# psy-ex/svt-av1-psy

Measured on AMD Instinct MI355X. Metric: Mblocks/s per kernel (SAD, FwdTxfm2d, CDEF) + encoder fps @1080p preset 8, higher is better.
Workload: dtype u8

## Files before the change

### svt-av1-psy_amd/csrc/sad.hip

```cpp
#include "svt_hip_common.h"
#include "../../include/svtav1_hip.h"
#include "hme_geom.h"
#include <vector>

namespace {

struct __attribute__((packed, aligned(4))) U64A4 { unsigned long long v; };
struct __attribute__((aligned(4))) u32x4_a4 { uint32_t x, y, z, w; };
struct __attribute__((aligned(16))) u32x4_a16 { uint32_t x, y, z, w; };

constexpr uint32_t MAX_SAD_VALUE = 128 * 128 * 255;
constexpr int      ME_TW         = 64;
constexpr int      ME_TH         = 32;
constexpr int      KEY_POS_BITS  = 11;
constexpr uint32_t ME_WAVE_MAX_W = 24, ME_WAVE_MAX_H = 16;

__device__ __forceinline__ void stage_rows_u8(uint32_t* lds, int pitch_dw, const uint8_t* g, uint32_t gstride, int width,
                                              int rows, int tid, int nthreads) {
    const int total = rows * pitch_dw;
    for (int i = tid; i < total; i += nthreads) {
        const int r   = i / pitch_dw;
        const int k   = i - r * pitch_dw;
        const int col = k * 4;
        uint32_t  v   = 0;
        if (col < width) {
            const uint8_t*  p    = g + (size_t)r * gstride + col;
            const uint32_t  sh   = (uint32_t)((uintptr_t)p & 3);
            const uint32_t* ap   = (const uint32_t*)(p - sh);
            const int       need = (width - col) < 4 ? (width - col) : 4;
            const uint32_t  lo   = ap[0];
            uint32_t        hi   = 0;
            if ((int)sh + need > 4) hi = ap[1];
            v = __builtin_amdgcn_alignbyte(hi, lo, sh);
            if (need < 4) v &= (1u << (8 * need)) - 1u;
        }
        lds[i] = v;
    }
}

struct __attribute__((packed, aligned(1))) u32x4_a1 { uint32_t x, y, z, w; };
struct __attribute__((packed, aligned(1))) u32_a1 { uint32_t x; };
struct __attribute__((aligned(8))) u32x2_a8 { uint32_t x, y; };

template <int NIT, int CL2>
__device__ __forceinline__ void stage_rows_load(uint32_t (&v)[NIT][4], const uint8_t* g, uint32_t gstride, int width, int rows, int tid) {
#pragma unroll
    for (int k = 0; k < NIT; ++k) {
        const int  idx = tid + 256 * k, r = idx >> CL2, col = (idx & ((1 << CL2) - 1)) * 16;
        const bool live = r < rows && col < width;
        const int  left = width - col;
        const int  back = (live && left < 16) ? 16 - left : 0;
        const uint8_t* p = g + (live ? (size_t)r * gstride + (size_t)(col - back) : (size_t)0);
        const u32x4_a1 t = *(const u32x4_a1*)p;
        v[k][0] = t.x; v[k][1] = t.y; v[k][2] = t.z; v[k][3] = t.w;
    }
#pragma unroll
    for (int k = 0; k < NIT; ++k) {
        const int  idx = tid + 256 * k, r = idx >> CL2, col = (idx & ((1 << CL2) - 1)) * 16;
        const bool live = r < rows && col < width;
        const int  left = width - col;
        uint32_t   x0 = live ? v[k][0] : 0u, x1 = live ? v[k][1] : 0u, x2 = live ? v[k][2] : 0u, x3 = live ? v[k][3] : 0u;
        if (live && left < 16) {
            const int back = 16 - left;
            if (back & 4) { x0 = x1; x1 = x2; x2 = x3; x3 = 0; }
            if (back & 8) { x0 = x2; x1 = x3; x2 = 0; x3 = 0; }
            const uint32_t bs = (uint32_t)back & 3u;
            x0 = __builtin_amdgcn_alignbyte(x1, x0, bs);
            x1 = __builtin_amdgcn_alignbyte(x2, x1, bs);
            x2 = __builtin_amdgcn_alignbyte(x3, x2, bs);
            x3 = __builtin_amdgcn_alignbyte(0u, x3, bs);
        }
        v[k][0] = x0; v[k][1] = x1; v[k][2] = x2; v[k][3] = x3;
    }
}
template <int NIT, int CL2>
__device__ __forceinline__ void stage_rows_store(const uint32_t (&v)[NIT][4], uint32_t* lds, int pitch_dw, int rows, int tid) {
#pragma unroll
    for (int k = 0; k < NIT; ++k) {
        const int idx = tid + 256 * k, r = idx >> CL2, c4 = (idx & ((1 << CL2) - 1)) * 4;
        if (r < rows) {
            uint32_t* o = lds + r * pitch_dw + c4;
            if (c4 + 0 < pitch_dw) *(u32x2_a8*)(o + 0) = u32x2_a8{v[k][0], v[k][1]};
            if (c4 + 2 < pitch_dw) *(u32x2_a8*)(o + 2) = u32x2_a8{v[k][2], v[k][3]};
        }
    }
}

template <int NT, int U>
__device__ __forceinline__ void stage_rows_wide_step(uint32_t* lds, const int pitch_dw, const uint8_t* g, const uint32_t gstride, const int width, const int total,
                                                     const int cpr, const int dr, const int dc, const int base, const int tid, int& r, int& c) {
    uint32_t v[U][4];
    int      rk[U], ck[U];
#pragma unroll
    for (int k = 0; k < U; ++k) {
        const int  idx = base + tid + NT * k, col = c * 16;
        rk[k] = r; ck[k] = c;
        const bool live = idx < total && col < width;
        const int  left = width - col;
        const int  back = (live && left < 16) ? 16 - left : 0;
        const uint8_t* p = g + (live ? (uint32_t)r * gstride + (uint32_t)(col - back) : 0u);
        const u32x4_a1 t = *(const u32x4_a1*)p;
        uint32_t x0 = live ? t.x : 0u, x1 = live ? t.y : 0u, x2 = live ? t.z : 0u, x3 = live ? t.w : 0u;
        if (back) {
            if (back & 4) { x0 = x1; x1 = x2; x2 = x3; x3 = 0; }
            if (back & 8) { x0 = x2; x1 = x3; x2 = 0; x3 = 0; }
            const uint32_t bs = (uint32_t)back & 3u;
            x0 = __builtin_amdgcn_alignbyte(x1, x0, bs);
            x1 = __builtin_amdgcn_alignbyte(x2, x1, bs);
            x2 = __builtin_amdgcn_alignbyte(x3, x2, bs);
            x3 = __builtin_amdgcn_alignbyte(0u, x3, bs);
        }
        v[k][0] = x0; v[k][1] = x1; v[k][2] = x2; v[k][3] = x3;
        r += dr; c += dc;
        if (c >= cpr) { c -= cpr; r++; }
    }
#pragma unroll
    for (int k = 0; k < U; ++k) {
        const int idx = base + tid + NT * k, c4 = ck[k] * 4;
        if (idx < total) {
            uint32_t* o = lds + rk[k] * pitch_dw + c4;
            if (c4 + 0 < pitch_dw) *(u32x2_a8*)(o + 0) = u32x2_a8{v[k][0], v[k][1]};
            if (c4 + 2 < pitch_dw) *(u32x2_a8*)(o + 2) = u32x2_a8{v[k][2], v[k][3]};
        }
    }
}
template <int NT = 256>
__device__ __forceinline__ void stage_rows_wide_any(uint32_t* lds, int pitch_dw, const uint8_t* g, uint32_t gstride, int width, int rows, int tid) {
    const int cpr = (pitch_dw + 3) >> 2, total = rows * cpr;
    const int dr = NT / cpr, dc = NT - dr * cpr;
    int       r = tid / cpr, c = tid - r * cpr;
    int base = 0;
    for (; total - base > 2 * NT; base += 4 * NT) stage_rows_wide_step<NT, 4>(lds, pitch_dw, g, gstride, width, total, cpr, dr, dc, base, tid, r, c);
    if (total - base > NT) stage_rows_wide_step<NT, 2>(lds, pitch_dw, g, gstride, width, total, cpr, dr, dc, base, tid, r, c);
    else if (total - base > 0) stage_rows_wide_step<NT, 1>(lds, pitch_dw, g, gstride, width, total, cpr, dr, dc, base, tid, r, c);
}

template <int NT>
__device__ __forceinline__ void stage_rows_wide_cpr(uint32_t* lds, int pitch_dw, const uint8_t* g, uint32_t gstride, int width, int rows, int cpr, int tid) {
    const int total = rows * cpr, dr = NT / cpr, dc = NT - dr * cpr;
    int       r = tid / cpr, c = tid - r * cpr, base = 0;
    for (; total - base > 2 * NT; base += 4 * NT) stage_rows_wide_step<NT, 4>(lds, pitch_dw, g, gstride, width, total, cpr, dr, dc, base, tid, r, c);
    if (total - base > NT) stage_rows_wide_step<NT, 2>(lds, pitch_dw, g, gstride, width, total, cpr, dr, dc, base, tid, r, c);
    else if (total - base > 0) stage_rows_wide_step<NT, 1>(lds, pitch_dw, g, gstride, width, total, cpr, dr, dc, base, tid, r, c);
}

__device__ __forceinline__ uint32_t dpp_add_quad_xor1(uint32_t v) {
    return v + (uint32_t)__builtin_amdgcn_update_dpp(0, (int)v, 0xB1, 0xf, 0xf, false);
}
__device__ __forceinline__ uint32_t dpp_add_quad_xor2(uint32_t v) {
    return v + (uint32_t)__builtin_amdgcn_update_dpp(0, (int)v, 0x4E, 0xf, 0xf, false);
}
__device__ __forceinline__ uint32_t dpp_add_row_ror4(uint32_t v) {
    return v + (uint32_t)__builtin_amdgcn_update_dpp(0, (int)v, 0x124, 0xf, 0xf, false);
}
__device__ __forceinline__ uint32_t dpp_add_row_ror8(uint32_t v) {
    return v + (uint32_t)__builtin_amdgcn_update_dpp(0, (int)v, 0x128, 0xf, 0xf, false);
}
__device__ __forceinline__ uint32_t umin32(uint32_t a, uint32_t b) { return a < b ? a : b; }


constexpr int ME_PITCH = 34;

template <bool SUB, bool FULL, int PITCH = ME_PITCH>
__device__ __forceinline__ void me_search_strips(const uint32_t* __restrict__ win, const uint32_t (&s)[8][2], int Wt, int Ht, int g0, int gstep, int l,
                                                 uint32_t& best8, uint32_t& best16, uint32_t& best32, uint32_t& best64) {
    const int bx = (l & 1) | ((l >> 1) & 2) | ((l >> 2) & 4);
    const int by = ((l >> 1) & 1) | ((l >> 2) & 2) | ((l >> 3) & 4);
    const int q  = l & 3;
    const int      G    = (Wt + 3) >> 2;
    const uint32_t qsel = 0x0c0c0100u + 0x0202u * (uint32_t)q;
    for (int g = g0; g < G; g += gstep) {
        const uint32_t* colp   = win + (by * 8) * PITCH + bx * 2 + g;
        const int       nvalid = (Wt - 4 * g) < 4 ? (Wt - 4 * g) : 4;
        const uint32_t inv1 = nvalid > 1 ? 0u : 0xffffffffu, inv2 = nvalid > 2 ? 0u : 0xffffffffu, inv3 = nvalid > 3 ? 0u : 0xffffffffu;
        const uint32_t invq = q < nvalid ? 0u : 0xffffffffu;
        U64A4 ra[8], rb[8];
#pragma unroll
        for (int r = 0; r < 7; r++) {
            ra[r] = *(const U64A4*)(colp + r * PITCH);
            rb[r] = *(const U64A4*)(colp + r * PITCH + 1);
        }
        uint32_t pos = (uint32_t)(4 * g), posq = (uint32_t)(4 * g + q);
        for (int yb = 0; yb < Ht; yb += 8) {
            const uint32_t* rowp = colp + (yb + 7) * PITCH;
#pragma unroll
            for (int i = 0; i < 8; i++) {
                if (yb + i < Ht) {
                    ra[(i + 7) & 7] = *(const U64A4*)(rowp + i * PITCH);
                    rb[(i + 7) & 7] = *(const U64A4*)(rowp + i * PITCH + 1);
                    unsigned long long acc = 0;
#pragma unroll
                    for (int r = 0; r < 8; r += (SUB ? 2 : 1)) {
                        acc = __builtin_amdgcn_qsad_pk_u16_u8(ra[(i + r) & 7].v, s[r][0], acc);
                        acc = __builtin_amdgcn_qsad_pk_u16_u8(rb[(i + r) & 7].v, s[r][1], acc);
                    }
                    if (SUB) acc <<= 1;
                    const uint32_t lo = (uint32_t)acc, hi = (uint32_t)(acc >> 32);
                    uint32_t k0 = (lo << 16) | pos, k1 = (lo & 0xffff0000u) | (pos + 1), k2 = (hi << 16) | (pos + 2),
                             k3 = (hi & 0xffff0000u) | (pos + 3);
                    if (!FULL) { k1 |= inv1; k2 |= inv2; k3 |= inv3; }
                    best8 = umin32(umin32(best8, k0), k1);
                    best8 = umin32(umin32(best8, k2), k3);
                    const uint32_t tlo = dpp_add_quad_xor2(dpp_add_quad_xor1(lo));
                    const uint32_t thi = dpp_add_quad_xor2(dpp_add_quad_xor1(hi));
                    const uint32_t sad16 = __builtin_amdgcn_perm(thi, tlo, qsel);
                    const uint32_t pq    = FULL ? posq : (posq | invq);
                    best16 = umin32(best16, (sad16 << KEY_POS_BITS) | pq);
                    const uint32_t sad32 = dpp_add_row_ror8(dpp_add_row_ror4(sad16));
                    best32 = umin32(best32, (sad32 << KEY_POS_BITS) | pq);
                    const auto     x16   = __builtin_amdgcn_permlane16_swap(sad32, sad32, false, false);
                    const uint32_t pair  = x16[0] + x16[1];
                    const auto     x32   = __builtin_amdgcn_permlane32_swap(pair, pair, false, false);
                    const uint32_t sad64 = x32[0] + x32[1];
                    best64 = umin32(best64, (sad64 << KEY_POS_BITS) | pq);
                    pos += ME_TW;
                    posq += ME_TW;
                }
            }
        }
    }
}

template <bool SUB>
__global__ __launch_bounds__(256, 4) void me_fullpel_kernel(const uint8_t* __restrict__ src_base, const uint8_t* __restrict__ ref_base,
                                                         const SvtHipMeSearchDesc* __restrict__ descs, uint32_t n,
                                                         uint32_t tiles_x,
                                                         uint32_t* __restrict__ best_sad, uint32_t* __restrict__ best_mv,
                                                         unsigned long long* __restrict__ keys) {
    HIP_DYNAMIC_SHARED(uint32_t, smem)
    uint32_t* src_lds  = smem;
    uint32_t* best_lds = smem + 64 * 16;
    uint32_t* win      = smem + 64 * 16 + 88;

    const int      tid  = threadIdx.x;
    const uint32_t item = xcd_remap(blockIdx.x, n);
    const uint32_t tile = blockIdx.y;
    const SvtHipMeSearchDesc d = descs[item];
    const int W   = d.search_area_width, H = d.search_area_height;
    const int tx0 = (int)(tile % tiles_x) * ME_TW;
    const int ty0 = (int)(tile / tiles_x) * ME_TH;
    if (tx0 >= W || ty0 >= H) {
        if (tile == 0 && keys == nullptr && tid < SVT_HIP_ME_NUM_BLOCKS) {
            best_sad[(size_t)item * SVT_HIP_ME_NUM_BLOCKS + tid] = MAX_SAD_VALUE;
            best_mv[(size_t)item * SVT_HIP_ME_NUM_BLOCKS + tid]  = 0;
        }
        return;
    }
    const int Wt = (W - tx0) < ME_TW ? (W - tx0) : ME_TW;
    const int Ht = (H - ty0) < ME_TH ? (H - ty0) : ME_TH;

    {
        uint32_t vs[1][4], vw[3][4];
        stage_rows_load<1, 2>(vs, src_base + d.src_off, d.src_stride, 64, 64, tid);
        stage_rows_load<3, 3>(vw, ref_base + d.ref_off + (size_t)ty0 * d.ref_stride + tx0, d.ref_stride, 64 + Wt - 1, 64 + Ht - 1, tid);
        stage_rows_store<1, 2>(vs, src_lds, 16, 64, tid);
        stage_rows_store<3, 3>(vw, win, ME_PITCH, 64 + Ht - 1, tid);
    }
    if (tid < 88) best_lds[tid] = 0xffffffffu;
    __syncthreads();

    const int l  = tid & 63;
    const int wv = tid >> 6;
    uint32_t s[8][2];
    {
        const int bx = (l & 1) | ((l >> 1) & 2) | ((l >> 2) & 4);
        const int by = ((l >> 1) & 1) | ((l >> 2) & 2) | ((l >> 3) & 4);
#pragma unroll
        for (int r = 0; r < 8; r++) {
            s[r][0] = src_lds[(by * 8 + r) * 16 + bx * 2 + 0];
            s[r][1] = src_lds[(by * 8 + r) * 16 + bx * 2 + 1];
        }
    }
    uint32_t best8 = 0xffffffffu, best16 = 0xffffffffu, best32 = 0xffffffffu, best64 = 0xffffffffu;
    if ((Wt & 3) == 0) me_search_strips<SUB, true>(win, s, Wt, Ht, wv, 4, l, best8, best16, best32, best64);
    else me_search_strips<SUB, false>(win, s, Wt, Ht, wv, 4, l, best8, best16, best32, best64);

    atomicMin(&best_lds[21 + l], best8);
    atomicMin(&best_lds[5 + (l >> 2)], best16);
    atomicMin(&best_lds[1 + (l >> 4)], best32);
    atomicMin(&best_lds[0], best64);
    __syncthreads();
    if (tid < SVT_HIP_ME_NUM_BLOCKS) {
        const uint32_t key = best_lds[tid];
        const uint32_t sad = tid >= 21 ? (key >> 16) : (key >> KEY_POS_BITS);
        const int      X   = tx0 + (int)(key & 63u);
        const int      Y   = ty0 + (int)((key >> 6) & 31u);
        const size_t   o   = (size_t)item * SVT_HIP_ME_NUM_BLOCKS + tid;
        if (keys == nullptr) {
            best_sad[o] = sad;
            best_mv[o]  = ((uint32_t)(uint16_t)(Y + d.y_search_area_origin) << 16) | (uint16_t)(X + d.x_search_area_origin);
        } else {
            atomicMin(&keys[o], ((unsigned long long)sad << 32) | (unsigned long long)(uint32_t)(Y * W + X));
        }
    }
}

struct __attribute__((packed, aligned(1))) u32x2_a1 { uint32_t x, y; };
__device__ __forceinline__ uint32_t dpp_min_quad_xor1(uint32_t v) { return umin32(v, (uint32_t)__builtin_amdgcn_update_dpp(-1, (int)v, 0xB1, 0xf, 0xf, false)); }
__device__ __forceinline__ uint32_t dpp_min_quad_xor2(uint32_t v) { return umin32(v, (uint32_t)__builtin_amdgcn_update_dpp(-1, (int)v, 0x4E, 0xf, 0xf, false)); }
__device__ __forceinline__ uint32_t dpp_min_row_ror4(uint32_t v) { return umin32(v, (uint32_t)__builtin_amdgcn_update_dpp(-1, (int)v, 0x124, 0xf, 0xf, false)); }
__device__ __forceinline__ uint32_t dpp_min_row_ror8(uint32_t v) { return umin32(v, (uint32_t)__builtin_amdgcn_update_dpp(-1, (int)v, 0x128, 0xf, 0xf, false)); }

template <bool SUB, int PITCH>
__global__ __launch_bounds__(256) void me_fullpel_wave_kernel(const uint8_t* __restrict__ src_base, const uint8_t* __restrict__ ref_base,
                                                              const SvtHipMeSearchDesc* __restrict__ descs, const uint32_t n, const int win_dw,
                                                              uint32_t* __restrict__ best_sad, uint32_t* __restrict__ best_mv) {
    HIP_DYNAMIC_SHARED(uint32_t, smem)
    const int      l    = threadIdx.x & 63, wv = __builtin_amdgcn_readfirstlane((int)(threadIdx.x >> 6));
    const uint32_t item = xcd_remap(blockIdx.x, gridDim.x) * 4 + (uint32_t)wv;
    if (item >= n) return;
    const SvtHipMeSearchDesc d = descs[item];
    const int    W = d.search_area_width, H = d.search_area_height;
    const size_t o = (size_t)item * SVT_HIP_ME_NUM_BLOCKS;
    if (W <= 0 || H <= 0) {
        for (int k = l; k < SVT_HIP_ME_NUM_BLOCKS; k += 64) { best_sad[o + k] = MAX_SAD_VALUE; best_mv[o + k] = 0; }
        return;
    }
    uint32_t* win = smem + wv * win_dw;
    const int bx = (l & 1) | ((l >> 1) & 2) | ((l >> 2) & 4);
    const int by = ((l >> 1) & 1) | ((l >> 2) & 2) | ((l >> 3) & 4);
    uint32_t  s[8][2];
    {
        const uint8_t* sp = src_base + d.src_off + (size_t)(by * 8) * d.src_stride + bx * 8;
#pragma unroll
        for (int r = 0; r < 8; r++) {
            const u32x2_a1 t = *(const u32x2_a1*)(sp + (size_t)r * d.src_stride);
            s[r][0] = t.x; s[r][1] = t.y;
        }
    }
    const int width = 64 + W - 1;
    stage_rows_wide_cpr<64>(win, PITCH, ref_base + d.ref_off, d.ref_stride, width, 64 + H - 1, (width + 15) >> 4, l);
    __builtin_amdgcn_wave_barrier();

    uint32_t best8 = 0xffffffffu, best16 = 0xffffffffu, best32 = 0xffffffffu, best64 = 0xffffffffu;
    if ((W & 3) == 0) me_search_strips<SUB, true, PITCH>(win, s, W, H, 0, 1, l, best8, best16, best32, best64);
    else me_search_strips<SUB, false, PITCH>(win, s, W, H, 0, 1, l, best8, best16, best32, best64);
    best16 = dpp_min_quad_xor2(dpp_min_quad_xor1(best16));
    best32 = dpp_min_row_ror8(dpp_min_row_ror4(dpp_min_quad_xor2(dpp_min_quad_xor1(best32))));
    best64 = dpp_min_row_ror8(dpp_min_row_ror4(dpp_min_quad_xor2(dpp_min_quad_xor1(best64))));
    best64 = umin32(best64, (uint32_t)__shfl_xor((int)best64, 16));
    best64 = umin32(best64, (uint32_t)__shfl_xor((int)best64, 32));
    const int xo = d.x_search_area_origin, yo = d.y_search_area_origin;
    auto emit = [&](const int idx, const uint32_t key, const bool is8) {
        const uint32_t sad = is8 ? (key >> 16) : (key >> KEY_POS_BITS);
        const int      X = (int)(key & 63u), Y = (int)((key >> 6) & 31u);
        best_sad[o + idx] = sad;
        best_mv[o + idx]  = ((uint32_t)(uint16_t)(Y + yo) << 16) | (uint16_t)(X + xo);
    };
    emit(21 + l, best8, true);
    if ((l & 3) == 0) emit(5 + (l >> 2), best16, false);
    if ((l & 15) == 0) emit(1 + (l >> 4), best32, false);
    if (l == 0) emit(0, best64, false);
}

__global__ void me_finalize_kernel(const SvtHipMeSearchDesc* __restrict__ descs, uint32_t n, const unsigned long long* __restrict__ keys,
                                   uint32_t* __restrict__ best_sad, uint32_t* __restrict__ best_mv) {
    const uint32_t i = blockIdx.x * blockDim.x + threadIdx.x;
    if (i >= n * SVT_HIP_ME_NUM_BLOCKS) return;
    const SvtHipMeSearchDesc d   = descs[i / SVT_HIP_ME_NUM_BLOCKS];
    const unsigned long long key = keys[i];
    if (key == ~0ull) {
        best_sad[i] = MAX_SAD_VALUE;
        best_mv[i]  = 0;
        return;
    }
    const uint32_t pos = (uint32_t)key;
    const int      W   = d.search_area_width;
    const int      X = (int)(pos % (uint32_t)W), Y = (int)(pos / (uint32_t)W);
    best_sad[i]        = (uint32_t)(key >> 32);
    best_mv[i]         = ((uint32_t)(uint16_t)(Y + d.y_search_area_origin) << 16) | (uint16_t)(X + d.x_search_area_origin);
}

__device__ __forceinline__ uint32_t wave_sum(uint32_t v) {
    v += (uint32_t)__shfl_xor((int)v, 32);
    v += (uint32_t)__shfl_xor((int)v, 16);
    v = dpp_add_row_ror8(v);
    v = dpp_add_row_ror4(v);
    v = dpp_add_quad_xor2(v);
    v = dpp_add_quad_xor1(v);
    return v;
}

template <int CHUNK>
__device__ __forceinline__ uint32_t sad_chunks(const uint8_t* __restrict__ src, const uint8_t* __restrict__ ref, uint32_t ss, uint32_t rs,
                                               int cpr, int cshift, int total, int l) {
    uint32_t sad = 0;
    for (int i0 = l; i0 < total; i0 += 256) {
        uint32_t av[4][CHUNK / 4], bv[4][CHUNK / 4];
#pragma unroll
        for (int k = 0; k < 4; ++k) {
            const int  i  = i0 + 64 * k;
            const bool in = i < total;
            const int  r  = cshift >= 0 ? (i >> cshift) : (i / cpr);
            const int  c  = i - r * cpr;
            const uint8_t* pa = src + (size_t)r * ss + c * CHUNK;
            const uint8_t* pb = ref + (size_t)r * rs + c * CHUNK;
            if (CHUNK == 16) {
                u32x4_a1 a = {0, 0, 0, 0}, b = {0, 0, 0, 0};
                if (in) { a = *(const u32x4_a1*)pa; b = *(const u32x4_a1*)pb; }
                av[k][0] = a.x; av[k][CHUNK / 4 > 1 ? 1 : 0] = a.y; av[k][CHUNK / 4 > 2 ? 2 : 0] = a.z; av[k][CHUNK / 4 > 3 ? 3 : 0] = a.w;
                bv[k][0] = b.x; bv[k][CHUNK / 4 > 1 ? 1 : 0] = b.y; bv[k][CHUNK / 4 > 2 ? 2 : 0] = b.z; bv[k][CHUNK / 4 > 3 ? 3 : 0] = b.w;
            } else {
                u32_a1 a = {0}, b = {0};
                if (in) { a = *(const u32_a1*)pa; b = *(const u32_a1*)pb; }
                av[k][0] = a.x; bv[k][0] = b.x;
            }
        }
#pragma unroll
        for (int k = 0; k < 4; ++k)
#pragma unroll
            for (int j = 0; j < CHUNK / 4; ++j) sad = __builtin_amdgcn_sad_u8(av[k][j], bv[k][j], sad);
    }
    return sad;
}

__global__ __launch_bounds__(256) void sad_nxm_kernel(const uint8_t* __restrict__ src_base, const uint8_t* __restrict__ ref_base,
                                                      const SvtHipSadPair* __restrict__ pairs, uint32_t n, int width, int height,
                                                      uint32_t* __restrict__ sad_out) {
    const int      l    = threadIdx.x & 63;
    const uint32_t pair = xcd_remap(blockIdx.x, gridDim.x) * 4 + (threadIdx.x >> 6);
    if (pair >= n) return;
    const SvtHipSadPair p   = pairs[pair];
    const uint8_t*      src = src_base + p.src_off;
    const uint8_t*      ref = ref_base + p.ref_off;
    uint32_t            sad = 0;
    if ((width & 15) == 0) {
        const int cpr = width >> 4;
        sad = sad_chunks<16>(src, ref, p.src_stride, p.ref_stride, cpr, (cpr & (cpr - 1)) ? -1 : __builtin_ctz(cpr), cpr * height, l);
    } else if ((width & 3) == 0) {
        const int cpr = width >> 2;
        sad = sad_chunks<4>(src, ref, p.src_stride, p.ref_stride, cpr, (cpr & (cpr - 1)) ? -1 : __builtin_ctz(cpr), cpr * height, l);
    } else {
        const int total = width * height;
        for (int i = l; i < total; i += 64) {
            const int r = i / width, c = i - r * width;
            const int a = src[(size_t)r * p.src_stride + c], b = ref[(size_t)r * p.ref_stride + c];
            sad += (uint32_t)(a > b ? a - b : b - a);
        }
    }
    sad = wave_sum(sad);
    if (l == 0) sad_out[pair] = sad;
}

constexpr int SADP_PPW = 4;
struct SadRegs { uint32_t a[4][4], b[4][4]; };
__device__ __forceinline__ void sadp_issue(SadRegs& r, const uint8_t* __restrict__ src, const uint8_t* __restrict__ ref, const SvtHipSadPair& p, const int cpr,
                                           const int cshift, const int total, const int l) {
#pragma unroll
    for (int k = 0; k < 4; ++k) {
        const int  i  = l + 64 * k;
        const bool in = i < total;
        const int  rr = i >> cshift, c = i - (rr << cshift);
        u32x4_a1 a = {0, 0, 0, 0}, b = {0, 0, 0, 0};
        if (in) {
            a = *(const u32x4_a1*)(src + p.src_off + (size_t)rr * p.src_stride + c * 16);
            b = *(const u32x4_a1*)(ref + p.ref_off + (size_t)rr * p.ref_stride + c * 16);
        }
        r.a[k][0] = a.x; r.a[k][1] = a.y; r.a[k][2] = a.z; r.a[k][3] = a.w;
        r.b[k][0] = b.x; r.b[k][1] = b.y; r.b[k][2] = b.z; r.b[k][3] = b.w;
    }
}
__device__ __forceinline__ uint32_t sadp_reduce(const SadRegs& r) {
    uint32_t sad = 0;
#pragma unroll
    for (int k = 0; k < 4; ++k)
#pragma unroll
        for (int j = 0; j < 4; ++j) sad = __builtin_amdgcn_sad_u8(r.a[k][j], r.b[k][j], sad);
    return wave_sum(sad);
}
__global__ __launch_bounds__(256) void sad_nxm_pipe_kernel(const uint8_t* __restrict__ src_base, const uint8_t* __restrict__ ref_base,
                                                           const SvtHipSadPair* __restrict__ pairs, uint32_t n, int cshift , int total,
                                                           uint32_t* __restrict__ sad_out) {
    const int      l     = threadIdx.x & 63, w = __builtin_amdgcn_readfirstlane(threadIdx.x >> 6);
    const uint32_t first = xcd_remap(blockIdx.x, gridDim.x) * (4 * SADP_PPW) + (uint32_t)w;
    if (first >= n) return;
    const int cpr = 1 << cshift;
    SadRegs   cur, nxt;
    sadp_issue(cur, src_base, ref_base, pairs[first], cpr, cshift, total, l);
#pragma unroll
    for (int k = 0; k < SADP_PPW; ++k) {
        const uint32_t pair = first + 4u * (uint32_t)k, np = pair + 4u;
        const bool     more = k + 1 < SADP_PPW && np < n;
        if (more) sadp_issue(nxt, src_base, ref_base, pairs[np], cpr, cshift, total, l);
        const uint32_t sad = sadp_reduce(cur);
        if (l == 0) sad_out[pair] = sad;
        if (!more) break;
        cur = nxt;
    }
}

constexpr int SADS_SPW = 4;
struct StripRegs { uint32_t a[4][4], b[4][4]; };
__device__ __forceinline__ void strip_issue(StripRegs& r, const uint8_t* __restrict__ sp, const uint8_t* __restrict__ rp, const uint32_t ss, const uint32_t rs,
                                            const int row0, const int ro, const int height, const bool live) {
#pragma unroll
    for (int k = 0; k < 4; ++k) {
        const int row = row0 + 4 * k;
        u32x4_a1  a = {0, 0, 0, 0}, b = {0, 0, 0, 0};
        if (live && row + ro < height) {
            a = *(const u32x4_a1*)(sp + (size_t)row * ss);
            b = *(const u32x4_a1*)(rp + (size_t)row * rs);
        }
        r.a[k][0] = a.x; r.a[k][1] = a.y; r.a[k][2] = a.z; r.a[k][3] = a.w;
        r.b[k][0] = b.x; r.b[k][1] = b.y; r.b[k][2] = b.z; r.b[k][3] = b.w;
    }
}
__device__ __forceinline__ uint32_t strip_consume(const StripRegs& r, uint32_t sad) {
#pragma unroll
    for (int k = 0; k < 4; ++k)
#pragma unroll
        for (int j = 0; j < 4; ++j) sad = __builtin_amdgcn_sad_u8(r.a[k][j], r.b[k][j], sad);
    return sad;
}
__global__ __launch_bounds__(256) void sad_nxm_strip_kernel(const uint8_t* __restrict__ src_base, const uint8_t* __restrict__ ref_base,
                                                            const SvtHipSadPair* __restrict__ pairs, const uint32_t n, const int cshift ,
                                                            const int height, uint32_t* __restrict__ sad_out) {
    const int      l = threadIdx.x & 63, w = __builtin_amdgcn_readfirstlane(threadIdx.x >> 6);
    const int      cpr = 1 << cshift, nb = 16 >> cshift;
    const int      sb = (l & 15) >> cshift, j = l & (cpr - 1), ro = l >> 4;
    const int      groups = (height + 15) >> 4;
    const uint32_t strip0 = (xcd_remap(blockIdx.x, gridDim.x) * 4 + (uint32_t)w) * SADS_SPW;
    if (strip0 * (uint32_t)nb >= n) return;
    const uint8_t *sp = nullptr, *rp = nullptr;
    uint32_t       ss = 0, rs = 0;
    bool           live = false;
    auto open_strip = [&](const int k) {
        const uint32_t pair = (strip0 + (uint32_t)k) * (uint32_t)nb + (uint32_t)sb;
        live = k < SADS_SPW && pair < n;
        if (live) {
            const SvtHipSadPair p = pairs[pair];
            sp = src_base + p.src_off + (size_t)ro * p.src_stride + j * 16;
            rp = ref_base + p.ref_off + (size_t)ro * p.ref_stride + j * 16;
            ss = p.src_stride; rs = p.ref_stride;
        }
    };
    StripRegs cur, nxt;
    open_strip(0);
    strip_issue(cur, sp, rp, ss, rs, 0, ro, height, live);
    for (int k = 0; k < SADS_SPW; ++k) {
        if ((strip0 + (uint32_t)k) * (uint32_t)nb >= n) break;
        const bool     mine = live;
        uint32_t       sad  = 0;
        const uint32_t out  = (strip0 + (uint32_t)k) * (uint32_t)nb + (uint32_t)sb;
        for (int g = 0; g < groups; ++g) {
            if (g + 1 < groups) {
                strip_issue(nxt, sp, rp, ss, rs, 16 * (g + 1), ro, height, live);
            } else {
                open_strip(k + 1);
                strip_issue(nxt, sp, rp, ss, rs, 0, ro, height, live);
            }
            sad = strip_consume(cur, sad);
            cur = nxt;
        }
        for (int m = 1; m < cpr; m <<= 1) sad += (uint32_t)__shfl_xor((int)sad, m);
        sad += (uint32_t)__shfl_xor((int)sad, 16);
        sad += (uint32_t)__shfl_xor((int)sad, 32);
        if (mine && j == 0 && ro == 0) sad_out[out] = sad;
    }
}

__global__ __launch_bounds__(64) void sad_16b_kernel(const uint16_t* __restrict__ src, uint32_t src_stride, const uint16_t* __restrict__ ref,
                                                     uint32_t ref_stride, int width, int height, uint32_t* __restrict__ out) {
    const int l     = threadIdx.x;
    uint32_t  sad   = 0;
    const int total = width * height;
    for (int i = l; i < total; i += 64) {
        const int r = i / width, c = i - r * width;
        const int a = src[(size_t)r * src_stride + c], b = ref[(size_t)r * ref_stride + c];
        sad += (uint32_t)(a > b ? a - b : b - a);
    }
    sad = wave_sum(sad);
    if (l == 0) out[0] = sad;
}

template <int LXG>
__device__ __forceinline__ void sad_loop_item(uint32_t* smem, unsigned long long& wg_best, const uint8_t* __restrict__ src_base,
                                              const uint8_t* __restrict__ ref_base, const SvtHipSadLoopDesc& d, const uint32_t item, const uint32_t tile,
                                              const uint32_t tiles_x, unsigned long long* __restrict__ keys) {
    constexpr int TW = 4 << LXG, TH = 256 >> LXG;
    const int tid = threadIdx.x;
    const int W = d.search_area_width, H = d.search_area_height;
    const int bw = d.block_width, bh = d.block_height;
    const int tx0 = (int)(tile % tiles_x) * TW, ty0 = (int)(tile / tiles_x) * TH;
    if (tx0 >= W || ty0 >= H) return;
    const int Wt = (W - tx0) < TW ? (W - tx0) : TW;
    const int Ht = (H - ty0) < TH ? (H - ty0) : TH;
    const int src_pitch = ((bw + 15) >> 4) << 2;
    const int win_w     = bw + Wt - 1;
    const int win_pitch = (((bw + TW + 3) >> 2) + 3) & ~1;
    uint32_t* src_lds   = smem;
    uint32_t* win       = smem + src_pitch * bh;
    stage_rows_u8(src_lds, src_pitch, src_base + d.src_off, d.src_stride, bw, bh, tid, 256);
    if (tid == 0) wg_best = ~0ull;
    const int rstep    = (int)(d.ref_stride / d.src_stride_raw);
    const int win_rows = Ht + rstep * (bh - 1);
    const uint8_t* wsrc = ref_base + d.ref_off + (size_t)ty0 * d.src_stride_raw + tx0;
    if (win_w >= 16) stage_rows_wide_any(win, win_pitch, wsrc, d.src_stride_raw, win_w, win_rows, tid);
    else stage_rows_u8(win, win_pitch, wsrc, d.src_stride_raw, win_w, win_rows, tid, 256);
    __syncthreads();

    const int gx = tid & ((1 << LXG) - 1), yy = tid >> LXG;
    const bool skip_rule = (bw == 16) && (bh <= 16) && d.skip_search_line;
    unsigned long long best = ~0ull;
    if (yy < Ht && 4 * gx < Wt && !(skip_rule && (((ty0 + yy) & 1) == 0))) {
        uint32_t sad[4] = {0, 0, 0, 0};
        const int full_dw = bw >> 2, tail = bw & 3;
        for (int y = 0; y < bh; y++) {
            const uint32_t* rrow = win + (yy + rstep * y) * win_pitch + gx;
            const uint32_t* srow = src_lds + y * src_pitch;
            unsigned long long acc = 0;
            uint32_t prev = rrow[0];
            int      k    = 0;
            for (; k + 4 <= full_dw; k += 4) {
                const u32x4_a16 sv = *(const u32x4_a16*)(srow + k);
                const U64A4     n0 = *(const U64A4*)(rrow + k + 1), n1 = *(const U64A4*)(rrow + k + 3);
                const uint32_t  r1 = (uint32_t)n0.v, r2 = (uint32_t)(n0.v >> 32), r3 = (uint32_t)n1.v, r4 = (uint32_t)(n1.v >> 32);
                acc  = __builtin_amdgcn_qsad_pk_u16_u8(((unsigned long long)r1 << 32) | prev, sv.x, acc);
                acc  = __builtin_amdgcn_qsad_pk_u16_u8(n0.v, sv.y, acc);
                acc  = __builtin_amdgcn_qsad_pk_u16_u8(((unsigned long long)r3 << 32) | r2, sv.z, acc);
                acc  = __builtin_amdgcn_qsad_pk_u16_u8(n1.v, sv.w, acc);
                prev = r4;
                if ((k & 12) == 12) {
                    sad[0] += (uint32_t)acc & 0xffffu; sad[1] += (uint32_t)(acc >> 16) & 0xffffu;
                    sad[2] += (uint32_t)(acc >> 32) & 0xffffu; sad[3] += (uint32_t)(acc >> 48);
                    acc = 0;
                }
            }
            for (; k < full_dw; k++) {
                const uint32_t next = rrow[k + 1];
                acc  = __builtin_amdgcn_qsad_pk_u16_u8(((unsigned long long)next << 32) | prev, srow[k], acc);
                prev = next;
            }
            sad[0] += (uint32_t)acc & 0xffffu; sad[1] += (uint32_t)(acc >> 16) & 0xffffu;
            sad[2] += (uint32_t)(acc >> 32) & 0xffffu; sad[3] += (uint32_t)(acc >> 48);
// ... 984 lines not shown
```

Baseline: 23460.

## Batch 32x32 SAD reductions across four rows and specialize wave window staging

The ME search loop now gathers four row positions of 16x16 SADs and combines them with one DPP scatter-sum sequence (inline asm), instead of doing a separate row_ror reduction for every row. This lowers the per-row DPP and cross-lane cost of the 32x32 and 64x64 reductions. Lane-dependent position bits are added once at the end. Window staging is replaced by a wave-specialized routine with fixed column counts and a realigned tail load. It adds hand-written asm with hazard nops and more complex position encoding, which raises correctness risk.

```diff
diff --git a/svt-av1-psy_amd/csrc/sad.hip b/svt-av1-psy_amd/csrc/sad.hip
--- a/svt-av1-psy_amd/csrc/sad.hip
+++ b/svt-av1-psy_amd/csrc/sad.hip
@@ -135,15 +135,6 @@
     else if (total - base > 0) stage_rows_wide_step<NT, 1>(lds, pitch_dw, g, gstride, width, total, cpr, dr, dc, base, tid, r, c);
 }
 
-template <int NT>
-__device__ __forceinline__ void stage_rows_wide_cpr(uint32_t* lds, int pitch_dw, const uint8_t* g, uint32_t gstride, int width, int rows, int cpr, int tid) {
-    const int total = rows * cpr, dr = NT / cpr, dc = NT - dr * cpr;
-    int       r = tid / cpr, c = tid - r * cpr, base = 0;
-    for (; total - base > 2 * NT; base += 4 * NT) stage_rows_wide_step<NT, 4>(lds, pitch_dw, g, gstride, width, total, cpr, dr, dc, base, tid, r, c);
-    if (total - base > NT) stage_rows_wide_step<NT, 2>(lds, pitch_dw, g, gstride, width, total, cpr, dr, dc, base, tid, r, c);
-    else if (total - base > 0) stage_rows_wide_step<NT, 1>(lds, pitch_dw, g, gstride, width, total, cpr, dr, dc, base, tid, r, c);
-}
-
 __device__ __forceinline__ uint32_t dpp_add_quad_xor1(uint32_t v) {
     return v + (uint32_t)__builtin_amdgcn_update_dpp(0, (int)v, 0xB1, 0xf, 0xf, false);
 }
@@ -160,15 +151,43 @@
 
 
 constexpr int ME_PITCH = 34;
+
+__device__ __forceinline__ uint32_t dpp_scatter_sum_quads(const uint32_t (&v)[4]) {
+#ifdef SVT_HIP_EMU
+    const uint32_t a0 = dpp_add_row_ror8(v[0]), a1 = dpp_add_row_ror8(v[1]), a2 = dpp_add_row_ror8(v[2]), a3 = dpp_add_row_ror8(v[3]);
+    const uint32_t t0 = (uint32_t)__builtin_amdgcn_update_dpp((int)a0, (int)a2, 0xE4, 0xf, 0xc, false);
+    const uint32_t t1 = (uint32_t)__builtin_amdgcn_update_dpp((int)a1, (int)a3, 0xE4, 0xf, 0xc, false);
+    const uint32_t y  = (uint32_t)__builtin_amdgcn_update_dpp((int)t0, (int)t1, 0xE4, 0xf, 0xa, false);
+    const uint32_t x  = y + (uint32_t)__builtin_amdgcn_update_dpp(0, (int)t0, 0x12C, 0xf, 0x5, false);
+    return x + (uint32_t)__builtin_amdgcn_update_dpp(0, (int)t1, 0x124, 0xf, 0xa, false);
+#else
+    uint32_t t0, t1;
+    asm("s_nop 1\n\t"
+        "v_add_u32_dpp %0, %2, %2 row_ror:8 row_mask:0xf bank_mask:0x3\n\t"
+        "v_add_u32_dpp %0, %4, %4 row_ror:8 row_mask:0xf bank_mask:0xc\n\t"
+        "v_add_u32_dpp %1, %3, %3 row_ror:8 row_mask:0xf bank_mask:0x3\n\t"
+        "v_add_u32_dpp %1, %5, %5 row_ror:8 row_mask:0xf bank_mask:0xc\n\t"
+        "v_add_u32_dpp %0, %0, %0 row_ror:12 row_mask:0xf bank_mask:0x5\n\t"
+        "s_nop 0\n\t"
+        "v_add_u32_dpp %0, %1, %1 row_ror:4 row_mask:0xf bank_mask:0xa"
+        : "=&v"(t0), "=&v"(t1)
+        : "v"(v[0]), "v"(v[1]), "v"(v[2]), "v"(v[3]));
+    return t0;
+#endif
+}
 
 template <bool SUB, bool FULL, int PITCH = ME_PITCH>
 __device__ __forceinline__ void me_search_strips(const uint32_t* __restrict__ win, const uint32_t (&s)[8][2], int Wt, int Ht, int g0, int gstep, int l,
                                                  uint32_t& best8, uint32_t& best16, uint32_t& best32, uint32_t& best64) {
     const int bx = (l & 1) | ((l >> 1) & 2) | ((l >> 2) & 4);
     const int by = ((l >> 1) & 1) | ((l >> 2) & 2) | ((l >> 3) & 4);
-    const int q  = l & 3;
+    const int q  = l & 3, c = (l >> 2) & 3;
     const int      G    = (Wt + 3) >> 2;
     const uint32_t qsel = 0x0c0c0100u + 0x0202u * (uint32_t)q;
+    uint32_t       himask = 0xffff0000u;
+    SVT_HIP_OPAQUE_I32(himask);
+    constexpr uint32_t NO_STEP = 0x1ffffu;
+    uint32_t       b16 = 0xffffffffu, b32 = 0xffffffffu, b64 = 0xffffffffu;
     for (int g = g0; g < G; g += gstep) {
         const uint32_t* colp   = win + (by * 8) * PITCH + bx * 2 + g;
         const int       nvalid = (Wt - 4 * g) < 4 ? (Wt - 4 * g) : 4;
@@ -180,45 +199,56 @@
             ra[r] = *(const U64A4*)(colp + r * PITCH);
             rb[r] = *(const U64A4*)(colp + r * PITCH + 1);
         }
-        uint32_t pos = (uint32_t)(4 * g), posq = (uint32_t)(4 * g + q);
+        uint32_t pos = (uint32_t)(4 * g);
         for (int yb = 0; yb < Ht; yb += 8) {
             const uint32_t* rowp = colp + (yb + 7) * PITCH;
 #pragma unroll
-            for (int i = 0; i < 8; i++) {
-                if (yb + i < Ht) {
-                    ra[(i + 7) & 7] = *(const U64A4*)(rowp + i * PITCH);
-                    rb[(i + 7) & 7] = *(const U64A4*)(rowp + i * PITCH + 1);
-                    unsigned long long acc = 0;
-#pragma unroll
-                    for (int r = 0; r < 8; r += (SUB ? 2 : 1)) {
-                        acc = __builtin_amdgcn_qsad_pk_u16_u8(ra[(i + r) & 7].v, s[r][0], acc);
-                        acc = __builtin_amdgcn_qsad_pk_u16_u8(rb[(i + r) & 7].v, s[r][1], acc);
+            for (int h = 0; h < 2; h++) {
+                if (yb + 4 * h < Ht) {
+                    uint32_t v[4] = {NO_STEP, NO_STEP, NO_STEP, NO_STEP};
+#pragma unroll
+                    for (int j = 0; j < 4; j++) {
+                        const int i = 4 * h + j;
+                        if (yb + i < Ht) {
+                            ra[(i + 7) & 7] = *(const U64A4*)(rowp + i * PITCH);
+                            rb[(i + 7) & 7] = *(const U64A4*)(rowp + i * PITCH + 1);
+                            unsigned long long acc = 0;
+#pragma unroll
+                            for (int r = 0; r < 8; r += (SUB ? 2 : 1)) {
+                                acc = __builtin_amdgcn_qsad_pk_u16_u8(ra[(i + r) & 7].v, s[r][0], acc);
+                                acc = __builtin_amdgcn_qsad_pk_u16_u8(rb[(i + r) & 7].v, s[r][1], acc);
+                            }
+                            if (SUB) acc <<= 1;
+                            const uint32_t lo = (uint32_t)acc, hi = (uint32_t)(acc >> 32);
+                            const uint32_t p1 = FULL ? pos + 1 : ((pos + 1) | inv1), p2 = FULL ? pos + 2 : ((pos + 2) | inv2), p3 = FULL ? pos + 3 : ((pos + 3) | inv3);
+                            const uint32_t k0 = (lo << 16) | pos, k1 = (lo & himask) | p1, k2 = (hi << 16) | p2, k3 = (hi & himask) | p3;
+                            best8 = umin32(umin32(best8, k0), k1);
+                            best8 = umin32(umin32(best8, k2), k3);
+                            const uint32_t tlo = dpp_add_quad_xor2(dpp_add_quad_xor1(lo));
+                            const uint32_t thi = dpp_add_quad_xor2(dpp_add_quad_xor1(hi));
+                            v[j] = __builtin_amdgcn_perm(thi, tlo, qsel);
+                            const uint32_t k16 = (v[j] << KEY_POS_BITS) | pos;
+                            b16 = umin32(b16, FULL ? k16 : (k16 | invq));
+                            pos += ME_TW;
+                        }
                     }
-                    if (SUB) acc <<= 1;
-                    const uint32_t lo = (uint32_t)acc, hi = (uint32_t)(acc >> 32);
-                    uint32_t k0 = (lo << 16) | pos, k1 = (lo & 0xffff0000u) | (pos + 1), k2 = (hi << 16) | (pos + 2),
-                             k3 = (hi & 0xffff0000u) | (pos + 3);
-                    if (!FULL) { k1 |= inv1; k2 |= inv2; k3 |= inv3; }
-                    best8 = umin32(umin32(best8, k0), k1);
-                    best8 = umin32(umin32(best8, k2), k3);
-                    const uint32_t tlo = dpp_add_quad_xor2(dpp_add_quad_xor1(lo));
-                    const uint32_t thi = dpp_add_quad_xor2(dpp_add_quad_xor1(hi));
-                    const uint32_t sad16 = __builtin_amdgcn_perm(thi, tlo, qsel);
-                    const uint32_t pq    = FULL ? posq : (posq | invq);
-                    best16 = umin32(best16, (sad16 << KEY_POS_BITS) | pq);
-                    const uint32_t sad32 = dpp_add_row_ror8(dpp_add_row_ror4(sad16));
-                    best32 = umin32(best32, (sad32 << KEY_POS_BITS) | pq);
+                    const uint32_t gpos  = (uint32_t)(4 * g + ME_TW * (yb + 4 * h));
+                    const uint32_t sad32 = dpp_scatter_sum_quads(v);
+                    const uint32_t k32   = (sad32 << KEY_POS_BITS) | gpos;
+                    b32 = umin32(b32, FULL ? k32 : (k32 | invq));
                     const auto     x16   = __builtin_amdgcn_permlane16_swap(sad32, sad32, false, false);
                     const uint32_t pair  = x16[0] + x16[1];
                     const auto     x32   = __builtin_amdgcn_permlane32_swap(pair, pair, false, false);
                     const uint32_t sad64 = x32[0] + x32[1];
-                    best64 = umin32(best64, (sad64 << KEY_POS_BITS) | pq);
-                    pos += ME_TW;
-                    posq += ME_TW;
+                    const uint32_t k64   = (sad64 << KEY_POS_BITS) | gpos;
+                    b64 = umin32(b64, FULL ? k64 : (k64 | invq));
                 }
             }
         }
     }
+    best16 = umin32(best16, b16 | (uint32_t)q);
+    best32 = umin32(best32, b32 | (uint32_t)(q | (c << 6)));
+    best64 = umin32(best64, b64 | (uint32_t)(q | (c << 6)));
 }
 
 template <bool SUB>
@@ -301,6 +331,52 @@
 __device__ __forceinline__ uint32_t dpp_min_row_ror4(uint32_t v) { return umin32(v, (uint32_t)__builtin_amdgcn_update_dpp(-1, (int)v, 0x124, 0xf, 0xf, false)); }
 __device__ __forceinline__ uint32_t dpp_min_row_ror8(uint32_t v) { return umin32(v, (uint32_t)__builtin_amdgcn_update_dpp(-1, (int)v, 0x128, 0xf, 0xf, false)); }
 
+template <int NF, int PITCH>
+__device__ __forceinline__ void stage_window_wave(uint32_t* lds, const uint8_t* g, const uint32_t gstride, const int width, const int rows, const int l) {
+    constexpr int RPI = 64 / NF;
+    const int     rem = width & 15, back = 16 - rem;
+    const bool    p0 = rem != 0 && l < rows, p1 = rem != 0 && l + 64 < rows;
+    u32x4_a1      t[2] = {{0u, 0u, 0u, 0u}, {0u, 0u, 0u, 0u}};
+    const uint32_t tail_off = (uint32_t)l * gstride + (uint32_t)(width - 16);
+    if (p0) t[0] = *(const u32x4_a1*)(g + tail_off);
+    if (p1) t[1] = *(const u32x4_a1*)(g + (size_t)64 * gstride + tail_off);
+
+    const int lr = l / NF, lc = l - lr * NF;
+    if (lr < RPI) {
+        const uint32_t goff = (uint32_t)lr * gstride + (uint32_t)lc * 16u;
+        uint32_t*      lp   = lds + lr * PITCH + lc * 4;
+        for (int r0 = 0; r0 < rows; r0 += 4 * RPI) {
+            const uint8_t* gb = g + (size_t)r0 * gstride;
+            u32x4_a1       v[4];
+#pragma unroll
+            for (int k = 0; k < 4; k++)
+                if (r0 + k * RPI + lr < rows) v[k] = *(const u32x4_a1*)(gb + (size_t)(k * RPI) * gstride + goff);
+#pragma unroll
+            for (int k = 0; k < 4; k++)
+                if (r0 + k * RPI + lr < rows) {
+                    uint32_t* o = lp + (r0 + k * RPI) * PITCH;
+                    *(u32x2_a8*)(o + 0) = u32x2_a8{v[k].x, v[k].y};
+                    *(u32x2_a8*)(o + 2) = u32x2_a8{v[k].z, v[k].w};
+                }
+        }
+    }
+#pragma unroll
+    for (int k = 0; k < 2; k++)
+        if (k == 0 ? p0 : p1) {
+            uint32_t x0 = t[k].x, x1 = t[k].y, x2 = t[k].z, x3 = t[k].w;
+            if (back & 4) { x0 = x1; x1 = x2; x2 = x3; x3 = 0; }
+            if (back & 8) { x0 = x2; x1 = x3; x2 = 0; x3 = 0; }
+            const uint32_t bs = (uint32_t)back & 3u;
+            x0 = __builtin_amdgcn_alignbyte(x1, x0, bs);
+            x1 = __builtin_amdgcn_alignbyte(x2, x1, bs);
+            x2 = __builtin_amdgcn_alignbyte(x3, x2, bs);
+            x3 = __builtin_amdgcn_alignbyte(0u, x3, bs);
+            uint32_t* o = lds + (l + 64 * k) * PITCH + NF * 4;
+            if (NF * 4 + 0 < PITCH) *(u32x2_a8*)(o + 0) = u32x2_a8{x0, x1};
+            if (NF * 4 + 2 < PITCH) *(u32x2_a8*)(o + 2) = u32x2_a8{x2, x3};
+        }
+}
+
 template <bool SUB, int PITCH>
 __global__ __launch_bounds__(256) void me_fullpel_wave_kernel(const uint8_t* __restrict__ src_base, const uint8_t* __restrict__ ref_base,
                                                               const SvtHipMeSearchDesc* __restrict__ descs, const uint32_t n, const int win_dw,
@@ -329,7 +405,8 @@
         }
     }
     const int width = 64 + W - 1;
-    stage_rows_wide_cpr<64>(win, PITCH, ref_base + d.ref_off, d.ref_stride, width, 64 + H - 1, (width + 15) >> 4, l);
+    if (PITCH >= 22 && (width >> 4) == 5) stage_window_wave<5, PITCH>(win, ref_base + d.ref_off, d.ref_stride, width, 64 + H - 1, l);
+    else stage_window_wave<4, PITCH>(win, ref_base + d.ref_off, d.ref_stride, width, 64 + H - 1, l);
     __builtin_amdgcn_wave_barrier();
 
     uint32_t best8 = 0xffffffffu, best16 = 0xffffffffu, best32 = 0xffffffffu, best64 = 0xffffffffu;
```

After: 26610 (median of 6 runs). +13.4%, better.
